# pmcgannon22/rlcard

Hardware: AMD Instinct MI355X
Metric: env-steps/s (whole node) + achieved HBM GB/s, leduc-holdem 1048576 envs/GPU (higher is better)
Workload: dtype int32

## Files before the change

rlcard_amd/csrc/cs_device.h:

```cpp
#pragma once
#include <hip/hip_runtime.h>
#include <stdint.h>
#include <type_traits>

#include "cs_prof.h"

namespace cs {

typedef uint32_t u32x4_t __attribute__((ext_vector_type(4)));
__device__ __forceinline__ void out_store16(uint4* p, const uint4& v)
{
    const u32x4_t x = {v.x, v.y, v.z, v.w};
    __builtin_nontemporal_store(x, (u32x4_t*)p);
}
template <class T>
__device__ __forceinline__ void out_store(T* p, T v)
{
    __builtin_nontemporal_store(v, p);
}

constexpr int MT_N = 624;
constexpr int MT_M = 397;
constexpr int WAVE = 64;

struct GameParams {
    int32_t num_players;
    int32_t num_decks;
    int32_t chips_for_each;
    int32_t dealer_id;
    int32_t rng_mode;
};

struct GameDefaults {
    static constexpr bool LANE_OPAQUE = true;
    static constexpr bool REWARD_OPAQUE = false;
    static constexpr bool PAYOFF_DRAWS = false;
    static constexpr int SPARSE_K = 0;
    static constexpr int MAX_POLICY = 0;
    static constexpr bool RANDOM_ACTIONS = false;
    static constexpr int DQ = 0;
    static constexpr bool OBS_DIRECT = false;
    static constexpr int RAW_SPAN_LEN = 0, RAW_SPAN_AT = 0;
};

__device__ __forceinline__ uint32_t mt_temper(uint32_t y)
{
    y ^= (y >> 11);
    y ^= (y << 7) & 0x9d2c5680u;
    y ^= (y << 15) & 0xefc60000u;
    y ^= (y >> 18);
    return y;
}

__device__ __forceinline__ uint32_t mt_temper_lo8(uint32_t y)
{
    y ^= (y >> 11);
    y ^= (y << 7) & 0x9d2c5680u;
    return y ^ (y >> 18) ^ ((y >> 3) & 0xF1u);
}

__device__ __forceinline__ uint32_t mt_mix(uint32_t cur, uint32_t nxt, uint32_t far)
{
    uint32_t y;
    asm("v_bfi_b32 %0, %1, %2, %3" : "=v"(y) : "s"(0x7fffffffu), "v"(nxt), "v"(cur));
    return far ^ (y >> 1) ^ ((0u - (nxt & 1u)) & 0x9908b0dfu);
}

template <class M>
__device__ __forceinline__ uint32_t mt_get(M mt, int k)
{
    if constexpr (std::is_pointer<M>::value) return mt[k];
    else return mt.get(k);
}
template <class M>
__device__ __forceinline__ void mt_set(M mt, int k, uint32_t v)
{
    if constexpr (std::is_pointer<M>::value) mt[k] = v;
    else mt.set(k, v);
}

template <class M>
__device__ inline void mt_init_by_array(M mt, const uint32_t* key, int klen)
{
    uint32_t prev = 19650218u;
    mt_set(mt, 0, prev);
    for (int i = 1; i < MT_N; i++) {
        prev = 1812433253u * (prev ^ (prev >> 30)) + (uint32_t)i;
        mt_set(mt, i, prev);
    }
    int i = 1, j = 0;
    prev = mt_get(mt, 0);
    for (int k = MT_N; k; k--) {
        const uint32_t v = (mt_get(mt, i) ^ ((prev ^ (prev >> 30)) * 1664525u)) + key[j] + (uint32_t)j;
        mt_set(mt, i, v);
        prev = v;
        i++;
        j++;
        if (i >= MT_N) { mt_set(mt, 0, mt_get(mt, MT_N - 1)); prev = mt_get(mt, 0); i = 1; }
        if (j >= klen) j = 0;
    }
    for (int k = MT_N - 1; k; k--) {
        const uint32_t v = (mt_get(mt, i) ^ ((prev ^ (prev >> 30)) * 1566083941u)) - (uint32_t)i;
        mt_set(mt, i, v);
        prev = v;
        i++;
        if (i >= MT_N) { mt_set(mt, 0, mt_get(mt, MT_N - 1)); prev = mt_get(mt, 0); i = 1; }
    }
    mt_set(mt, 0, 0x80000000u);
}

template <class M>
__device__ inline void mt_twist_inplace(M mt)
{
    for (int k = 0; k < MT_N - MT_M; k++) mt_set(mt, k, mt_mix(mt_get(mt, k), mt_get(mt, k + 1), mt_get(mt, k + MT_M)));
    for (int k = MT_N - MT_M; k < MT_N - 1; k++)
        mt_set(mt, k, mt_mix(mt_get(mt, k), mt_get(mt, k + 1), mt_get(mt, k + MT_M - MT_N)));
    mt_set(mt, MT_N - 1, mt_mix(mt_get(mt, MT_N - 1), mt_get(mt, 0), mt_get(mt, MT_M - 1)));
}

typedef __attribute__((address_space(1))) uint32_t gu32;
typedef __attribute__((address_space(1))) uint8_t gu8;

__device__ __forceinline__ gu32* lane_ptr(uint32_t* p, int j)
{
    const uint64_t b = (uint64_t)(uintptr_t)p;
    const uint64_t lo = (uint32_t)__builtin_amdgcn_readlane((int)(uint32_t)b, j);
    const uint64_t hi = (uint32_t)__builtin_amdgcn_readlane((int)(uint32_t)(b >> 32), j);
    return (gu32*)(uintptr_t)(lo | (hi << 32));
}

enum { STAGE_NONE = 0, STAGE_LDS = 2 };

template <int W, int PAD, int ROWS = WAVE>
struct Stage {
    static_assert(W % 16 == 0 && WAVE % (W / 4) == 0, "a staged row is copied by W / 4 lanes of one wave instruction");
    static_assert(PAD % 4 == 0, "rows are written as dwords");
    static constexpr int STRIDE = W + PAD;
    static constexpr int CHUNK = STRIDE % 16 == 0 ? 16 : (STRIDE % 8 == 0 ? 8 : 4);
    static constexpr int BYTES = ROWS * STRIDE + 16;
};

__device__ __forceinline__ void wave_sync_lds()
{
    __builtin_amdgcn_wave_barrier();
    __builtin_amdgcn_fence(__ATOMIC_RELEASE, "wavefront");
    __builtin_amdgcn_fence(__ATOMIC_ACQUIRE, "wavefront");
}

template <int W, int PAD>
__device__ __forceinline__ void stage_rows_copy(uint8_t* area, uint8_t* hbm_rows, int lane, int nvalid, bool to_lds)
{
    constexpr int STRIDE = Stage<W, PAD>::STRIDE, CH = Stage<W, PAD>::CHUNK, CPR = W / CH;
#pragma unroll
    for (int i = 0; i < CPR; i++) {
        const int q = i * WAVE + lane, row = q / CPR, col = q - row * CPR;
        if (row < nvalid) {
            uint8_t* l = area + row * STRIDE + col * CH;
            uint8_t* g = hbm_rows + (size_t)q * CH;
            if constexpr (CH == 16) {
                if (to_lds) *(uint4*)l = *(const uint4*)g;
                else *(uint4*)g = *(const uint4*)l;
            } else if constexpr (CH == 8) {
                if (to_lds) *(uint2*)l = *(const uint2*)g;
                else *(uint2*)g = *(const uint2*)l;
            } else {
                if (to_lds) *(uint32_t*)l = *(const uint32_t*)g;
                else *(uint32_t*)g = *(const uint32_t*)l;
            }
        }
    }
    wave_sync_lds();
}

__device__ __forceinline__ void philox4(uint64_t seed, uint64_t env, uint64_t blk, uint32_t (&out)[4])
{
    uint32_t c0 = (uint32_t)env, c1 = (uint32_t)(env >> 32), c2 = (uint32_t)blk, c3 = (uint32_t)(blk >> 32);
    uint32_t k0 = (uint32_t)seed, k1 = (uint32_t)(seed >> 32);
#pragma unroll
    for (int r = 0; r < 10; r++) {
        const uint32_t hi0 = __umulhi(0xD2511F53u, c0), lo0 = 0xD2511F53u * c0;
        const uint32_t hi1 = __umulhi(0xCD9E8D57u, c2), lo1 = 0xCD9E8D57u * c2;
        const uint32_t n0 = hi1 ^ c1 ^ k0, n2 = hi0 ^ c3 ^ k1;
        c0 = n0;
        c1 = lo1;
        c2 = n2;
        c3 = lo0;
        k0 += 0x9E3779B9u;
        k1 += 0xBB67AE85u;
    }
    out[0] = c0;
    out[1] = c1;
    out[2] = c2;
    out[3] = c3;
}

__device__ __forceinline__ uint32_t philox_u32(uint64_t seed, uint64_t env, uint64_t t)
{
    uint32_t w[4];
    philox4(seed, env, t >> 2, w);
    const uint32_t q = (uint32_t)t & 3u;
    return q == 0 ? w[0] : (q == 1 ? w[1] : (q == 2 ? w[2] : w[3]));
}

struct PolicyRng {
    uint32_t w0, w1, w2, w3;
    __device__ __forceinline__ uint32_t at(uint64_t seed, uint64_t env, uint64_t t, bool first)
    {
        const uint32_t q = (uint32_t)t & 3u;
        if (first || q == 0) {
            uint32_t w[4];
            philox4(seed, env, t >> 2, w);
            w0 = w[0]; w1 = w[1]; w2 = w[2]; w3 = w[3];
        }
        return q == 0 ? w0 : (q == 1 ? w1 : (q == 2 ? w2 : w3));
    }
};

__device__ __forceinline__ int pick_legal32(uint32_t legal, uint32_t r)
{
    const int count = __popc(legal);
    if (count == 0) return -1;
    int k = (int)__umulhi(r, (uint32_t)count);
    while (k--) legal &= legal - 1;
    return __builtin_ctz(legal);
}
__device__ __forceinline__ int pick_legal64(uint64_t legal, uint32_t r)
{
    const int count = __popcll(legal);
    if (count == 0) return -1;
    int k = (int)__umulhi(r, (uint32_t)count);
    while (k--) legal &= legal - 1;
    return __builtin_ctzll(legal);
}
struct Legal128 {
    uint64_t lo, hi;
};
__device__ __forceinline__ bool legal_empty(const Legal128& m) { return (m.lo | m.hi) == 0ull; }
__device__ __forceinline__ bool legal_has(const Legal128& m, int a) { return ((a < 64 ? m.lo : m.hi) >> (a & 63)) & 1ull; }
__device__ __forceinline__ int legal_lowest(const Legal128& m)
{
    return m.lo ? __builtin_ctzll(m.lo) : 64 + __builtin_ctzll(m.hi);
}
__device__ __forceinline__ int pick_legal128(const Legal128& legal, uint32_t r)
{
    const int clo = __popcll(legal.lo), count = clo + __popcll(legal.hi);
    if (count == 0) return -1;
    int k = (int)__umulhi(r, (uint32_t)count);
    const bool high = k >= clo;
    uint64_t w = high ? legal.hi : legal.lo;
    k -= high ? clo : 0;
    while (k--) w &= w - 1;
    return (high ? 64 : 0) + __builtin_ctzll(w);
}
struct Legal256 {
    uint64_t w[4];
};
__device__ __forceinline__ bool legal_empty(const Legal256& m) { return (m.w[0] | m.w[1] | m.w[2] | m.w[3]) == 0ull; }
__device__ __forceinline__ uint64_t legal_word(const Legal256& m, int k)
{
    return k == 0 ? m.w[0] : (k == 1 ? m.w[1] : (k == 2 ? m.w[2] : m.w[3]));
}
__device__ __forceinline__ bool legal_has(const Legal256& m, int a) { return (legal_word(m, a >> 6) >> (a & 63)) & 1ull; }
__device__ __forceinline__ int legal_lowest(const Legal256& m)
{
    if (m.w[0]) return __builtin_ctzll(m.w[0]);
    if (m.w[1]) return 64 + __builtin_ctzll(m.w[1]);
    if (m.w[2]) return 128 + __builtin_ctzll(m.w[2]);
    return 192 + __builtin_ctzll(m.w[3]);
}
__device__ __forceinline__ int pick_legal256(const Legal256& legal, uint32_t r)
{
    const int c0 = __popcll(legal.w[0]), c1 = c0 + __popcll(legal.w[1]), c2 = c1 + __popcll(legal.w[2]);
    const int count = c2 + __popcll(legal.w[3]);
    if (count == 0) return -1;
    int k = (int)__umulhi(r, (uint32_t)count);
    const int q = k < c0 ? 0 : (k < c1 ? 1 : (k < c2 ? 2 : 3));
    uint64_t w = legal_word(legal, q);
    k -= q == 0 ? 0 : (q == 1 ? c0 : (q == 2 ? c1 : c2));
    while (k--) w &= w - 1;
    return 64 * q + __builtin_ctzll(w);
}
template <int A>
__device__ __forceinline__ int pick_legal_small(uint32_t legal, uint32_t r)
{
    static_assert(A >= 1 && A <= 8, "small action sets");
    const uint32_t count = (uint32_t)__popc(legal);
    const uint32_t k = __umulhi(r, count);
#pragma unroll
    for (uint32_t i = 0; i + 1 < (uint32_t)A; i++) legal = i < k ? legal & (legal - 1u) : legal;
    return count == 0 ? -1 : __builtin_ctz(legal);
}

template <int ROW, int ROWS = WAVE>
struct RowWriter {
    static_assert(ROW % 4 == 0, "byte rows must be dword multiples");
    static constexpr int DW = ROW / 4;
    static constexpr int LDS_WORDS = ROWS * DW;
    static constexpr int NB = (ROW + 31) / 32;
    static constexpr int Q = (ROWS * DW) / 4;

    __device__ static __forceinline__ uint32_t expand4(uint32_t x)
    {
        return __umul24(x & 15u, 0x204081u) & 0x01010101u;
    }

    __device__ static __forceinline__ void write(uint32_t* lds, const uint32_t (&bits)[NB], uint8_t* out_span,
                                                 int lane, int nvalid, bool wide = true)
    {
        if (lane < ROWS) {
#pragma unroll
            for (int j = 0; j < DW; j++) lds[lane * DW + j] = expand4(bits[j / 8] >> (4 * (j % 8)));
        }
        write_out(lds, bits, out_span, lane, nvalid, wide);
    }
    __device__ static __forceinline__ void write_out(uint32_t* lds, const uint32_t (&)[NB], uint8_t* out_span,
                                                     int lane, int nvalid, bool wide)
    {
        __builtin_amdgcn_wave_barrier();
        __builtin_amdgcn_fence(__ATOMIC_RELEASE, "wavefront");
        __builtin_amdgcn_fence(__ATOMIC_ACQUIRE, "wavefront");
        if (wide && nvalid == ROWS && (((uintptr_t)out_span) & 15u) == 0) {
            uint4* o = (uint4*)out_span;
            const uint4* src = (const uint4*)lds;
#pragma unroll
            for (int j = 0; j < (Q + WAVE - 1) / WAVE; j++) {
                const int q = j * WAVE + lane;
                if (q < Q) out_store16(o + q, src[q]);
            }
        } else {
            uint32_t* o = (uint32_t*)out_span;
            const int total = nvalid * DW;
#pragma unroll
            for (int j = 0; j < DW; j++) {
                const int e = j * WAVE + lane;
                if (e < total) o[e] = lds[e];
            }
        }
        __builtin_amdgcn_wave_barrier();
        __builtin_amdgcn_fence(__ATOMIC_RELEASE, "wavefront");
        __builtin_amdgcn_fence(__ATOMIC_ACQUIRE, "wavefront");
    }
};

template <int ROW, int ROWS = WAVE>
struct RowWriterRaw {
    static_assert(ROW % 2 == 0, "raw rows are staged as 16-bit pieces");
    static constexpr int NW = (ROW + 3) / 4;
    static constexpr int SPAN = ROWS * ROW;
    static constexpr int LDS_WORDS = (SPAN + 3) / 4;

    __device__ static __forceinline__ void write(uint32_t* lds, const uint32_t (&words)[NW], uint8_t* out_span,
                                                 int lane, int nvalid, bool wide = true)
    {
        if (lane < ROWS) {
            if constexpr (ROW % 4 == 0) {
#pragma unroll
                for (int j = 0; j < ROW / 4; j++) lds[lane * (ROW / 4) + j] = words[j];
            } else {
                uint16_t* l16 = (uint16_t*)lds + lane * (ROW / 2);
#pragma unroll
                for (int j = 0; j < ROW / 2; j++) l16[j] = (uint16_t)(words[j / 2] >> (16 * (j & 1)));
            }
        }
        write_out(lds, out_span, lane, nvalid, wide);
// ... 88 lines not shown
```

rlcard_amd/csrc/cs_leduc.h:

```cpp
#pragma once
#include "cs_device.h"
#include "../../include/cardsim.h"

#include "cs_prof.h"

namespace cs {

struct Leduc : GameDefaults {
    static constexpr int OBS = 36, A = 4, P = 2, LB = 1, WORDS = 2, ACTION_BYTES = 1;
    static constexpr int NB = 2;
    static constexpr bool RAW_OBS = false;
    static constexpr int SCRATCH_WORDS = 0;
    static constexpr int STAGE_W = 64, STAGE_PAD = 4, STAGE_R = 12;
    static constexpr int STAGE_RF = 24;
    static constexpr int RESTAGE_B = 4;
    static constexpr int MIN_WAVES = 6;
    static constexpr int EPW = 64;
    __device__ __forceinline__ void bind(uint32_t*, const GameParams&) {}
    enum { CALL = 0, RAISE = 1, FOLD = 2, CHECK = 3 };

    int h0, h1, pub, in0, in1, r0, r1, hr, nrn, over, rc, ptr, f0, f1;

    __device__ __forceinline__ void load(const uint32_t* st, int64_t n, int64_t env)
    {
        const uint32_t w0 = st[env], w1 = st[n + env];
        h0 = w0 & 7; h1 = (w0 >> 3) & 7; pub = (w0 >> 6) & 7; in0 = (w0 >> 9) & 31; in1 = (w0 >> 14) & 31;
        r0 = (w0 >> 19) & 15; r1 = (w0 >> 23) & 15; hr = (w0 >> 27) & 3; nrn = (w0 >> 29) & 3; over = w0 >> 31;
        rc = w1 & 3; ptr = (w1 >> 2) & 1; f0 = (w1 >> 3) & 1; f1 = (w1 >> 4) & 1;
    }
    __device__ __forceinline__ void store(uint32_t* st, int64_t n, int64_t env) const
    {
        st[env] = (uint32_t)h0 | (uint32_t)h1 << 3 | (uint32_t)pub << 6 | (uint32_t)in0 << 9 | (uint32_t)in1 << 14 |
                  (uint32_t)r0 << 19 | (uint32_t)r1 << 23 | (uint32_t)hr << 27 | (uint32_t)nrn << 29 |
                  (uint32_t)over << 31;
        st[n + env] = (uint32_t)rc | (uint32_t)ptr << 2 | (uint32_t)f0 << 3 | (uint32_t)f1 << 4;
    }
    __device__ __forceinline__ void blank() { h0 = h1 = pub = in0 = in1 = r0 = r1 = hr = nrn = rc = ptr = f0 = f1 = 0; over = 1; }

    __device__ __forceinline__ int current() const { return ptr; }
    __device__ __forceinline__ bool is_over() const { return over != 0; }

    __device__ __forceinline__ uint32_t legal() const
    {
        const int mx = r0 > r1 ? r0 : r1, rp = ptr ? r1 : r0;
        uint32_t m = 0xF;
        if (hr >= 2) m &= ~(1u << RAISE);
        if (rp < mx) m &= ~(1u << CHECK);
        if (rp == mx) m &= ~(1u << CALL);
        return m;
    }

    static constexpr int MAX_POLICY = CS_POLICY_RULE_V2;
    __device__ __forceinline__ int rule_action(uint32_t policy, int player, uint32_t lg) const
    {
        const int hand = player ? h1 : h0;
        const int v1 = (lg >> RAISE) & 1u ? RAISE : ((lg >> CALL) & 1u ? CALL : ((lg >> CHECK) & 1u ? CHECK : FOLD));
        const bool pairs = rc >= 1 && ((pub ^ hand) >> 1) == 0;
        const int v2 = pairs ? ((lg >> RAISE) & 1u ? RAISE : CALL) : FOLD;
        return policy == CS_POLICY_RULE_V2 ? v2 : v1;
    }

    __device__ __forceinline__ void observe(int player, uint32_t (&bits)[NB]) const
    {
        const int my = player ? in1 : in0, hand = player ? h1 : h0;
        uint64_t b = (1ull << (hand >> 1)) | (1ull << (my + 6)) | (1ull << (in0 + in1 - my + 21));
        if (rc >= 1) b |= 1ull << ((pub >> 1) + 3);
        bits[0] = (uint32_t)b;
        bits[1] = (uint32_t)(b >> 32);
    }

    static constexpr int SPARSE_K = 4;
    __device__ __forceinline__ uint32_t observe_pos(int player, uint32_t (&pos)[4]) const
    {
        const int my = player ? in1 : in0, hand = (player ? h1 : h0) >> 1;
        pos[0] = (uint32_t)hand;
        pos[1] = (uint32_t)(rc >= 1 ? (pub >> 1) + 3 : hand);
        pos[2] = (uint32_t)(my + 6);
        pos[3] = (uint32_t)(in0 + in1 - my + 21);
        return 0;
    }

    template <class Rng>
    __device__ __forceinline__ static bool deal_swar(Rng& rng, uint32_t& code)
    {
        const uint32_t k0 = rng.staged_offset();
        const uint32_t avail = k0 < rng.sn ? rng.sn - k0 : 0u, nv = avail < 16u ? avail : 16u;
        if (nv < 6u) return false;
        const uint32_t* row = (const uint32_t*)(rng.stg + (k0 & ~3u));
        uint32_t w[5];
#pragma unroll
        for (int i = 0; i < 5; i++) w[i] = row[i];
        uint32_t m0 = 0, m1 = 0, m3 = 0;
#pragma unroll
        for (int i = 0; i < 4; i++) {
            const uint32_t x = __builtin_amdgcn_alignbyte(w[i + 1], w[i], k0 & 3u);
            const uint32_t b1 = x >> 1, b2 = x >> 2;
            const uint32_t a0 = ~(b1 & b2) & 0x01010101u;
            const uint32_t a1 = ~(b2 & (b1 | x)) & 0x01010101u;
            const uint32_t a3 = ~(x & b1) & 0x01010101u;
            m0 |= ((a0 * 0x10204080u) >> 28) << (4 * i);
            m1 |= ((a1 * 0x10204080u) >> 28) << (4 * i);
            m3 |= ((a3 * 0x10204080u) >> 28) << (4 * i);
        }
        const uint32_t valid = (1u << nv) - 1u;
        m0 &= valid;
        if (!m0) return false;
        const uint32_t p0 = __builtin_ctz(m0);
        const uint32_t r1 = m1 & valid & (0xFFFFFFFEu << p0);
        if (!r1) return false;
        const uint32_t p1 = __builtin_ctz(r1), p2 = p1 + 1;
        const uint32_t r3 = m3 & valid & (0xFFFFFFFEu << p2);
        if (!r3) return false;
        const uint32_t p5 = __builtin_ctz(r3) + 2;
        if (p5 >= nv) return false;
        const uint8_t* b = rng.stg + k0;
        const uint32_t j1 = b[p0] & 7u, j2 = b[p1] & 7u, j3 = b[p2] & 3u, s = b[p5] & 1u;
        rng.advance_by(p5 + 1);
        const uint32_t hh0 = j1, hh1 = j2 == j1 ? 5u : j2;
        const uint32_t pb = j3 == j2 ? (j1 == 4u ? 5u : 4u) : (j3 == j1 ? 5u : j3);
        code = hh0 | hh1 << 3 | pb << 6 | s << 9;
        return true;
    }

    template <class Rng>
    __device__ __forceinline__ static uint32_t draw_deal(Rng& rng)
    {
#if CS_PROF_NO_RESET
        rng.advance_by(7u);
        return 0u | 2u << 3 | 4u << 6 | (rng.pos & 1u) << 9;
#endif
        if constexpr (Rng::kMode == STAGE_LDS) {
            uint32_t code;
            if (deal_swar(rng, code)) return code;
        }
        uint32_t deck = 0x543210u;
        uint32_t q = 0, s = 0;
        auto take = [&](uint32_t b) {
            const uint32_t mx = q < 5 ? 5 - q : 1;
            const uint32_t u = b & (mx >= 4 ? 7u : (mx >= 2 ? 3u : 1u));
            if (u <= mx) {
                if (q < 5) {
                    const uint32_t ci = (deck >> (4 * mx)) & 15u, cj = (deck >> (4 * u)) & 15u, x = ci ^ cj;
                    deck ^= (x << (4 * mx)) | (x << (4 * u));
                } else {
                    s = u;
                }
                q++;
            }
        };
        if constexpr (Rng::kMode == STAGE_LDS) {
            const uint32_t k0 = rng.staged_offset();
            uint32_t k = k0;
            while (q < 6 && k < rng.sn) {
                const uint32_t sh = k & 3u;
                const uint32_t w = *(const uint32_t*)(rng.stg + (k - sh)) >> (8 * sh);
#pragma unroll
                for (uint32_t t = 0; t < 4; t++)
                    if (t < 4 - sh && q < 6 && k < rng.sn) {
                        take((w >> (8 * t)) & 255u);
                        k++;
                    }
            }
            rng.advance_by(k - k0);
        }
        while (q < 6) take(rng.next8());
        return ((deck >> 20) & 15u) | ((deck >> 16) & 15u) << 3 | ((deck >> 12) & 15u) << 6 | s << 9;
    }

    __device__ __forceinline__ void deal_blinds(int s)
    {
        in0 = s == 0 ? 1 : 2;
        in1 = s == 0 ? 2 : 1;
        ptr = s;
        r0 = in0; r1 = in1;
        hr = 0; nrn = 0; rc = 0; f0 = 0; f1 = 0; over = 0;
    }

    template <class Rng>
    __device__ __forceinline__ void reset(Rng& rng)
    {
        const uint32_t e0 = draw_deal(rng);
        h0 = (int)(e0 & 7u);
        h1 = (int)((e0 >> 3) & 7u);
        pub = (int)((e0 >> 6) & 7u);
        deal_blinds((int)((e0 >> 9) & 1u));
    }

    template <class Rng>
    __device__ __forceinline__ void step(int a, Rng&)
    {
        const uint32_t lg = legal();
        if (a < 0 || a > 3 || !((lg >> a) & 1u)) a = ((lg >> CHECK) & 1u) ? CHECK : FOLD;
        const int mx = r0 > r1 ? r0 : r1, rp = ptr ? r1 : r0, ra = rc == 0 ? 2 : 4;
        int add = 0, nr = rp;
        if (a == CALL) { add = mx - rp; nr = mx; nrn += 1; }
        else if (a == RAISE) { add = mx - rp + ra; nr = mx + ra; hr += 1; nrn = 1; }
        else if (a == FOLD) { if (ptr) f1 = 1; else f0 = 1; }
        else { nrn += 1; }
        if (ptr) { in1 += add; r1 = nr; } else { in0 += add; r0 = nr; }
        ptr ^= 1;
        if (ptr ? f1 : f0) ptr ^= 1;
        if (nrn >= 2) {
            rc += 1;
            hr = 0; nrn = 0; r0 = 0; r1 = 0;
        }
        over = (f0 + f1 == 1) || rc >= 2;
    }

    __device__ __forceinline__ void payoffs(float (&r)[P]) const
    {
        int w0, w1;
        if (f0 || f1) { w0 = !f0; w1 = !f1; }
        else {
            const int pr = pub >> 1, k0 = h0 >> 1, k1 = h1 >> 1;
            if (k0 == pr) { w0 = 1; w1 = 0; }
            else if (k1 == pr) { w0 = 0; w1 = 1; }
            else { w0 = k0 >= k1; w1 = k1 >= k0; }
        }
        const float tot = (float)(in0 + in1), each = (w0 & w1) ? tot * 0.5f : tot;
        r[0] = (w0 ? each - (float)in0 : -(float)in0) * 0.5f;
        r[1] = (w1 ? each - (float)in1 : -(float)in1) * 0.5f;
    }
};

}
```

rlcard_amd/csrc/cs_prof.h:

```cpp
#pragma once

#ifndef CS_PROF_NO_OBS
#define CS_PROF_NO_OBS 0
#endif
#ifndef CS_PROF_NO_SMALL
#define CS_PROF_NO_SMALL 0
#endif
#ifndef CS_PROF_NO_RESET
#define CS_PROF_NO_RESET 0
#endif
#ifndef CS_PROF_NO_EVAL
#define CS_PROF_NO_EVAL 0
#endif
#ifndef CS_PROF_NO_DEAL9
#define CS_PROF_NO_DEAL9 0
#endif
#ifndef CS_PROF_NO_TRACK
#define CS_PROF_NO_TRACK 0
#endif
#ifndef CS_PROF_NO_SKIP
#define CS_PROF_NO_SKIP 0
#endif
#ifndef CS_PROF_MIXED_WRITER
#define CS_PROF_MIXED_WRITER 0
#endif
#ifndef CS_PROF_MIXED_NT
#define CS_PROF_MIXED_NT 0
#endif
#ifndef CS_PROF_BRIDGE_WAVES
#define CS_PROF_BRIDGE_WAVES 0
#endif
#ifndef CS_PROF_MIXED16_NT
#define CS_PROF_MIXED16_NT 0
#endif
#ifndef CS_PROF_SCOUT_MASK
#define CS_PROF_SCOUT_MASK 0
#endif
#ifndef CS_PROF_SCOUT_WAVES
#define CS_PROF_SCOUT_WAVES 0
#endif
#ifndef CS_PROF_DDZ
#define CS_PROF_DDZ 0
#endif
```

rlcard_amd/csrc/cs_skeleton.h:

```cpp
#pragma once
#include <cstddef>
#include <type_traits>

#include "cs_device.h"
#include "cs_ring.h"
#include "cs_engine.h"
#include "cs_dq.h"

namespace cs {

constexpr int BLOCK = 256;
constexpr int WAVES_PER_BLOCK = BLOCK / WAVE;

template <class G>
using legal_t = std::conditional_t<(G::A > 128), Legal256, std::conditional_t<(G::A > 64), Legal128, uint64_t>>;

struct LaneCtx {
    int lane, wid;
    int64_t env, wave_first;
    int nvalid;
    bool valid;
};

template <int EPW = WAVE>
// ... 428 lines not shown
    CS_SMEM(G);
    const LaneCtx c = lane_ctx(n);
    RingLane<> m = ring_lane(mt, ctl, c);
    G g;
    g.bind(scratch_of<G>(scr[c.wid], c.lane), prm);
    g.blank();
    float r[G::P];
#pragma unroll
    for (int k = 0; k < G::P; k++) r[k] = 0.f;
    bool done = false;
    if (c.valid) {
        g.load(st, n, c.env);
        if (g.is_over()) {
            game_reset(g, m, st, n, c.env);
        } else {
            g.step(actions[c.env], m);
            done = g.is_over();
            if (done) game_payoffs(g, r, m);
        }
    }
    refill(m, c.lane, flags & 1);
    uint32_t bits[G::NB];
    const int p = g.current();
    g.observe(p, bits);
    if (out.obs) emit_obs<G>(lds[c.wid], bits, (uint8_t*)out.obs, c.wave_first, flags, c);
    if (c.valid) {
        if (out.legal) emit_legal<G>((uint8_t*)out.legal, c.env, g.legal());
        if (out.player) ((uint8_t*)out.player)[c.env] = (uint8_t)p;
        if (out.reward) emit_reward<G>((float*)out.reward, c.env, r);
        if (out.done) ((uint8_t*)out.done)[c.env] = (uint8_t)done;
        g.store(st, n, c.env);
        ctl[c.env] = m.ctl_word();
    }
    step_record<G>(rec, st, n, c);
}

template <class G>
__global__ __launch_bounds__(BLOCK) void k_observe(const uint32_t* st, int64_t n, int player, cs_step_out out,
                                                    GameParams prm, StepRecord rec)
{
    CS_SMEM(G);
    const LaneCtx c = lane_ctx(n);
    G g;
    g.bind(scratch_of<G>(scr[c.wid], c.lane), prm);
    g.blank();
    if (c.valid) g.load(st, n, c.env);
    uint32_t bits[G::NB];
    g.observe(player, bits);
    if (out.obs) emit_obs<G>(lds[c.wid], bits, (uint8_t*)out.obs, c.wave_first, 0, c);
    if (c.valid) {
        if (out.legal) emit_legal<G>((uint8_t*)out.legal, c.env, g.legal());
        if (out.player) ((uint8_t*)out.player)[c.env] = (uint8_t)g.current();
        if (out.done) ((uint8_t*)out.done)[c.env] = (uint8_t)g.is_over();
    }
    step_record<G>(rec, st, n, c);
}

struct RolloutArgs {
    uint32_t* mt;
    uint32_t* ctl;
    uint32_t* st;
    int64_t n;
    uint64_t seed, t0, env_base;
    cs_traj_out out;
    GameParams prm;
    uint32_t* sctl;
    uint8_t* sbuf;
    int32_t T, flags;
    uint32_t seats;
    uint32_t pad_;
};
typedef const __attribute__((address_space(4))) RolloutArgs* RolloutArgsK;
static_assert(std::is_standard_layout<RolloutArgs>::value && std::is_trivially_copyable<RolloutArgs>::value,
              "RolloutArgs is copied into the kernarg segment bytewise");
static_assert(offsetof(RolloutArgs, mt) == 0 && alignof(RolloutArgs) == 8 && sizeof(RolloutArgs) % 8 == 0,
              "RolloutArgs: first kernarg at offset 0, 8-byte aligned");

template <class G, bool POL = false>
__global__ __launch_bounds__(BLOCK, G::MIN_WAVES) void k_rollout(RolloutArgs args)
{
    RolloutArgsK ak = (RolloutArgsK)__builtin_amdgcn_kernarg_segment_ptr();
    auto arg = [&]() -> const RolloutArgs& {
        asm volatile("" : "+s"(ak));
        return *(const RolloutArgs*)ak;
    };
    uint32_t* const mt = args.mt;
    uint32_t* const ctl = args.ctl;
    uint32_t* const st = args.st;
    const int64_t n = args.n;
    const int T = args.T, flags = args.flags;
    const GameParams prm = args.prm;
    uint32_t* const sctl = args.sctl;
    uint8_t* const sbuf = args.sbuf;
    CS_SMEM_ROWS(G, G::EPW);
    __shared__ __attribute__((aligned(16))) uint8_t stage[WAVES_PER_BLOCK][StageBytes<G>::value];
    const LaneCtx c = lane_ctx<G::EPW>(n);
    RingLane<STAGE_LDS> m = ring_lane<STAGE_LDS>(mt, ctl, c);
    const bool staged = !(flags & 3);
    uint8_t* rows = sbuf + c.wave_first * G::STAGE_W;
    if (staged) {
        if (c.valid && ((ctl[c.env] >> 17) & 1u)) {
            const uint32_t w = sctl[c.env];
            m.sp = w & 0xFFFFu;
            m.sn = w >> 16;
        }
        stage_rows_copy<G::STAGE_W, G::STAGE_PAD>(stage[c.wid], rows, c.lane, c.nvalid, true);
    }
    constexpr int DQ = DqOf<G>::value, DQW = DqOf<G>::words;
    __shared__ uint32_t dql[DQ > 0 ? WAVES_PER_BLOCK * G::EPW * DQW : 1];
    DqMem q{};
    if constexpr (DQ > 0) {
        q = DqMem{dql + (c.wid * G::EPW + (c.lane < G::EPW ? c.lane : 0)) * DQW, 1};
        if (c.valid) {
#pragma unroll
            for (int w = 0; w < DQW; w++) q.set(w, st[(int64_t)(G::GW + w) * n + c.env]);
        }
    }
    G g;
    g.bind(scratch_of<G>(scr[c.wid], c.lane), prm);
    g.blank();
    if (c.valid) {
        g.load(st, n, c.env);
        if (g.is_over()) {
            if constexpr (DQ > 0) dq_reset(g, m, q);
            else g.reset(m);
        }
    }
    refill(m, c.lane, flags & 1);
    if (staged) restage<G>(m, stage[c.wid], c.lane, c.valid);
    PolicyRng pol;
    const uint64_t genv0 = args.env_base + (uint64_t)c.env;
    for (int t = 0; t < T; t++) {
        const RolloutArgs& A = arg();
        LaneCtx cl = c;
        if constexpr (G::LANE_OPAQUE) {
            int ol = c.lane;
            asm volatile("" : "+v"(ol));
            cl.lane = ol;
            cl.env = c.wave_first + ol;
        }
        const cs_traj_out& out = A.out;
        uint8_t* obs = (uint8_t*)out.obs;
        uint8_t* legal = (uint8_t*)out.legal;
        uint8_t* player = (uint8_t*)out.player;
        float* reward = (float*)out.reward;
        uint8_t* done_o = (uint8_t*)out.done;
        const uint64_t seed = A.seed, t0 = A.t0;

        const int64_t rowbase = (int64_t)t * n;
        const int p = g.current();
        const legal_t<G> lg = g.legal();
        uint32_t bits[G::NB];
        g.observe(p, bits);
        const uint32_t pr = pol.at(seed, genv0, t0 + (uint64_t)t, t == 0);
        int a;
        static_assert(G::A <= 256, "the policy pick takes a legal mask of one, two or four 64-bit words");
        if constexpr (G::A > 128) a = pick_legal256(lg, pr);
        else if constexpr (G::A > 64) a = pick_legal128(lg, pr);
        else if constexpr (G::A <= 8) a = pick_legal_small<G::A>((uint32_t)lg, pr);
        else if constexpr (G::A <= 32) a = pick_legal32((uint32_t)lg, pr);
        else a = pick_legal64(lg, pr);
        if constexpr (POL) {
            const uint32_t pid = (A.seats >> (8 * p)) & 0xFFu;
            int ra;
            if constexpr (G::A <= 32) ra = g.rule_action(pid, p, (uint32_t)lg);
            else ra = g.rule_action(pid, p, lg, pr);
            a = pid == (uint32_t)CS_POLICY_RANDOM ? a : ra;
        }
#if !CS_PROF_NO_OBS
        if constexpr (G::SPARSE_K > 0) {
            uint32_t pos[G::SPARSE_K];
            const uint32_t tail = g.observe_pos(p, pos);
            row_write_sparse<G::OBS, G::EPW, G::SPARSE_K, G::RAW_OBS>(
                lds[c.wid], pos, obs + (rowbase + c.wave_first) * G::OBS, cl.lane, c.nvalid, !(flags & 4), tail);
        } else {
            emit_obs<G, G::EPW>(lds[c.wid], bits, obs, rowbase + c.wave_first, flags, cl);
        }
#endif
        uint32_t zr = 0;
        asm volatile("" : "+v"(zr));
        float r[G::P];
#pragma unroll
        for (int k = 0; k < G::P; k++) r[k] = __uint_as_float(zr);
        bool done = false;
        if (c.valid) {
            const int64_t row = rowbase + cl.env;
#if !CS_PROF_NO_SMALL
            emit_legal<G>(legal, row, lg);
            out_store(player + row, (uint8_t)p);
#endif
            if constexpr (G::ACTION_BYTES == 1) out_store((uint8_t*)out.action + row, (uint8_t)a);
            else out_store((int16_t*)out.action + row, (int16_t)a);
            g.step(a, m);
            done = g.is_over();
            if (done) {
                game_payoffs(g, r, m);
                if (out.final_obs) {
#pragma unroll
                    for (int q = 0; q < G::P; q++) {
                        uint32_t fb[G::NB];
                        g.observe(q, fb);
                        write_obs_direct<G>((uint8_t*)out.final_obs + (row * G::P + q) * G::OBS, fb);
                    }
                }
            }
#if !CS_PROF_NO_SMALL
            emit_reward<G>(reward, row, r);
            out_store(done_o + row, (uint8_t)done);
#endif
            if constexpr (DQ == 0) {
                if (done) g.reset(m);
            }
        }
        if constexpr (DQ > 0) {
            constexpr uint32_t CM = (1u << DqOf<G>::cb) - 1u;
            if (__ballot(c.valid && done && (q.get(0) & CM) == 0u)) {
                if (c.valid && (q.get(0) & CM) < (uint32_t)DQ) dq_push(g, m, q);
            }
            if (c.valid && done) dq_reset(g, m, q);
        }
        refill(m, cl.lane, flags & 1);
        if (staged) restage<G>(m, stage[c.wid], cl.lane, c.valid);
    }
    bool keep = false;
    if (staged) {
        stage_rows_copy<G::STAGE_W, G::STAGE_PAD>(stage[c.wid], rows, c.lane, c.nvalid, false);
        keep = true;
    }
    if (c.valid) {
        g.store(st, n, c.env);
        if constexpr (DQ > 0) {
#pragma unroll
            for (int w = 0; w < DQW; w++) st[(int64_t)(G::GW + w) * n + c.env] = q.get(w);
        }
        ctl[c.env] = m.ctl_word() | ((uint32_t)keep << 17);
        if (keep) sctl[c.env] = m.sp | (m.sn << 16);
    }
}

template <class G>
__global__ __launch_bounds__(BLOCK) void k_policy_actions(const uint32_t* st, int64_t n, int policy, uint64_t seed,
                                                           uint64_t t, uint64_t env_base, int32_t* actions,
                                                           GameParams prm)
{
    const int64_t env = (int64_t)blockIdx.x * BLOCK + threadIdx.x;
    uint32_t* lane_scratch = nullptr;
    if constexpr (G::SCRATCH_WORDS > 0) {
        __shared__ uint32_t scr[WAVES_PER_BLOCK][Scratch<G>::WORDS];
        lane_scratch = scratch_of<G>(scr[threadIdx.x / WAVE], threadIdx.x & (WAVE - 1));
    }
    if (env >= n) return;
    G g;
    g.bind(lane_scratch, prm);
    g.blank();
    g.load(st, n, env);
    int a = -1;
    if (!g.is_over()) {
        if constexpr (G::A > 128) {
            static_assert(G::MAX_POLICY == 0, "rule policies take masks of at most two words");
            a = pick_legal256(g.legal(), philox_u32(seed, env_base + (uint64_t)env, t));
        } else if constexpr (G::A > 64) {
            const Legal128 lg = g.legal();
            const uint32_t pr = philox_u32(seed, env_base + (uint64_t)env, t);
            if constexpr (G::MAX_POLICY > 0) {
                if (policy == CS_POLICY_RANDOM) a = pick_legal128(lg, pr);
                else a = g.rule_action((uint32_t)policy, g.current(), lg, pr);
            } else {
                a = pick_legal128(lg, pr);
            }
        } else if constexpr (G::A <= 32) {
            const uint32_t lg = (uint32_t)g.legal();
            if (policy == CS_POLICY_RANDOM) a = pick_legal_small<G::A>(lg, philox_u32(seed, env_base + (uint64_t)env, t));
            else a = g.rule_action((uint32_t)policy, g.current(), lg);
        } else {
            const uint64_t lg = g.legal();
            const uint32_t pr = philox_u32(seed, env_base + (uint64_t)env, t);
            if constexpr (G::MAX_POLICY > 0) {
                if (policy == CS_POLICY_RANDOM) a = pick_legal64(lg, pr);
                else a = g.rule_action((uint32_t)policy, g.current(), lg, pr);
            } else {
                a = pick_legal64(lg, pr);
            }
        }
    }
    actions[env] = a;
}

static inline GameParams params_of(const Buffers& b)
{
    return GameParams{b.num_players, b.num_decks, b.chips_for_each, b.dealer_id, b.rng_mode};
}
static inline dim3 grid_for(int64_t n, int epw = WAVE)
{
    const int64_t per = (int64_t)WAVES_PER_BLOCK * epw;
    return dim3((unsigned)((n + per - 1) / per));
}

template <class G>
static hipError_t seed_g(const Buffers& b, const uint32_t* keys, const int32_t* klen, int64_t first, int64_t count,
                         hipStream_t s)
{
    hipLaunchKernelGGL(k_seed<G>, grid_for(count), dim3(BLOCK), 0, s, b.mt, b.ctl, b.state, b.n, keys, klen, first,
                       count, b.kernel_flags, params_of(b));
    return hipGetLastError();
}
template <class G>
static hipError_t reset_g(const Buffers& b, const cs_step_out& o, hipStream_t s)
{
    hipLaunchKernelGGL(k_reset<G>, grid_for(b.n), dim3(BLOCK), 0, s, b.mt, b.ctl, b.state, b.n, o, b.kernel_flags,
                       params_of(b), b.rec);
    return hipGetLastError();
}
template <class G>
static hipError_t step_g(const Buffers& b, const int32_t* a, const cs_step_out& o, hipStream_t s)
{
    hipLaunchKernelGGL(k_step<G>, grid_for(b.n), dim3(BLOCK), 0, s, b.mt, b.ctl, b.state, b.n, a, o, b.kernel_flags,
                       params_of(b), b.rec);
    return hipGetLastError();
}
template <class G>
static hipError_t observe_g(const Buffers& b, int32_t p, const cs_step_out& o, hipStream_t s)
{
    hipLaunchKernelGGL(k_observe<G>, grid_for(b.n), dim3(BLOCK), 0, s, b.state, b.n, p, o, params_of(b), b.rec);
    return hipGetLastError();
}
template <class G>
static hipError_t rollout_g(const Buffers& b, int32_t T, uint64_t seed, uint64_t t0, uint64_t env_base,
                            const cs_traj_out& o, hipStream_t s)
{
    const RolloutArgs a{b.mt, b.ctl, b.state, b.n, seed, t0, env_base, o, params_of(b), b.sctl, b.sbuf, T, b.kernel_flags};
    hipLaunchKernelGGL(k_rollout<G>, grid_for(b.n, G::EPW), dim3(BLOCK), 0, s, a);
    return hipGetLastError();
}

template <class G>
static hipError_t rollout_policy_g(const Buffers& b, int32_t T, uint64_t seed, uint64_t t0, uint64_t env_base,
                                   uint32_t seats, const cs_traj_out& o, hipStream_t s)
{
    const RolloutArgs a{b.mt, b.ctl, b.state, b.n, seed, t0, env_base, o, params_of(b), b.sctl, b.sbuf, T, b.kernel_flags,
                        seats, 0u};
    hipLaunchKernelGGL((k_rollout<G, true>), grid_for(b.n, G::EPW), dim3(BLOCK), 0, s, a);
    return hipGetLastError();
}
template <class G>
static hipError_t policy_actions_g(const Buffers& b, int32_t policy, uint64_t seed, uint64_t t, uint64_t env_base,
                                   int32_t* actions, hipStream_t s)
{
    hipLaunchKernelGGL(k_policy_actions<G>, dim3((unsigned)((b.n + BLOCK - 1) / BLOCK)), dim3(BLOCK), 0, s, b.state,
                       b.n, policy, seed, t, env_base, actions, params_of(b));
    return hipGetLastError();
}

template <class G>
static void fill_info(cs_game_info* info)
{
    info->obs_dim = G::OBS;
    info->num_actions = G::A;
    info->num_players = G::P;
    info->legal_bytes = G::LB;
    info->action_bytes = G::ACTION_BYTES;
    info->state_words = G::WORDS;
    info->action_feature_dim = G::A;
    info->rng_period = (int32_t)RING;
    info->deal_queue_depth = DqOf<G>::value;
    info->game_words = G::WORDS - DqOf<G>::words;
    info->envs_per_wave = G::EPW;
}

template <class G>
static const GameOps* ops_of()
{
    static const GameOps ops = [] {
        GameOps o{seed_g<G>, reset_g<G>, step_g<G>, observe_g<G>, rollout_g<G>, {}, G::STAGE_W,
                  RING_ENV_WORDS, false, false};
        fill_info<G>(&o.info);
// ... 14 lines not shown
```

Baseline: 75.19 billion.

## Branchless Leduc rules, 64-bit-window deal, wide-multiply Philox, profiling knockouts

Moves the Leduc step, legal, payoff and blind logic into a shared host/device rules header and rewrites them as branchless select chains. The staged deal scan now packs the 16-byte window into nibbles and searches all positions with one 64-bit mask per card instead of four per-dword loops with early exits. Philox can use a 64-bit product to get the high and low halves together, and Leduc enables this by default. It also adds compile-time profiling switches that stub out philox, pick, step, refill and restage, all off by default. The aim is less divergence and fewer ALU ops per step, with the risk that the branchless forms do more work on average.

```diff
diff --git a/rlcard_amd/csrc/cs_device.h b/rlcard_amd/csrc/cs_device.h
--- a/rlcard_amd/csrc/cs_device.h
+++ b/rlcard_amd/csrc/cs_device.h
@@ -35,6 +35,7 @@
     static constexpr bool LANE_OPAQUE = true;
     static constexpr bool REWARD_OPAQUE = false;
     static constexpr bool PAYOFF_DRAWS = false;
+    static constexpr bool PHILOX_WIDE = false;
     static constexpr int SPARSE_K = 0;
     static constexpr int MAX_POLICY = 0;
     static constexpr bool RANDOM_ACTIONS = false;
@@ -172,14 +173,22 @@
     wave_sync_lds();
 }
 
+template <bool WIDE = false>
 __device__ __forceinline__ void philox4(uint64_t seed, uint64_t env, uint64_t blk, uint32_t (&out)[4])
 {
     uint32_t c0 = (uint32_t)env, c1 = (uint32_t)(env >> 32), c2 = (uint32_t)blk, c3 = (uint32_t)(blk >> 32);
     uint32_t k0 = (uint32_t)seed, k1 = (uint32_t)(seed >> 32);
 #pragma unroll
     for (int r = 0; r < 10; r++) {
-        const uint32_t hi0 = __umulhi(0xD2511F53u, c0), lo0 = 0xD2511F53u * c0;
-        const uint32_t hi1 = __umulhi(0xCD9E8D57u, c2), lo1 = 0xCD9E8D57u * c2;
+        uint32_t hi0, lo0, hi1, lo1;
+        if constexpr (WIDE) {
+            const uint64_t p0 = (uint64_t)0xD2511F53u * c0, p1 = (uint64_t)0xCD9E8D57u * c2;
+            hi0 = (uint32_t)(p0 >> 32); lo0 = (uint32_t)p0;
+            hi1 = (uint32_t)(p1 >> 32); lo1 = (uint32_t)p1;
+        } else {
+            hi0 = __umulhi(0xD2511F53u, c0); lo0 = 0xD2511F53u * c0;
+            hi1 = __umulhi(0xCD9E8D57u, c2); lo1 = 0xCD9E8D57u * c2;
+        }
         const uint32_t n0 = hi1 ^ c1 ^ k0, n2 = hi0 ^ c3 ^ k1;
         c0 = n0;
         c1 = lo1;
@@ -204,12 +213,13 @@
 
 struct PolicyRng {
     uint32_t w0, w1, w2, w3;
+    template <bool WIDE = false>
     __device__ __forceinline__ uint32_t at(uint64_t seed, uint64_t env, uint64_t t, bool first)
     {
         const uint32_t q = (uint32_t)t & 3u;
         if (first || q == 0) {
             uint32_t w[4];
-            philox4(seed, env, t >> 2, w);
+            philox4<WIDE>(seed, env, t >> 2, w);
             w0 = w[0]; w1 = w[1]; w2 = w[2]; w3 = w[3];
         }
         return q == 0 ? w0 : (q == 1 ? w1 : (q == 2 ? w2 : w3));
diff --git a/rlcard_amd/csrc/cs_leduc.h b/rlcard_amd/csrc/cs_leduc.h
--- a/rlcard_amd/csrc/cs_leduc.h
+++ b/rlcard_amd/csrc/cs_leduc.h
@@ -3,10 +3,11 @@
 #include "../../include/cardsim.h"
 
 #include "cs_prof.h"
+#include "cs_leduc_rules.h"
 
 namespace cs {
 
-struct Leduc : GameDefaults {
+struct Leduc : GameDefaults, leduc::State {
     static constexpr int OBS = 36, A = 4, P = 2, LB = 1, WORDS = 2, ACTION_BYTES = 1;
     static constexpr int NB = 2;
     static constexpr bool RAW_OBS = false;
@@ -17,9 +18,8 @@
     static constexpr int MIN_WAVES = 6;
     static constexpr int EPW = 64;
     __device__ __forceinline__ void bind(uint32_t*, const GameParams&) {}
-    enum { CALL = 0, RAISE = 1, FOLD = 2, CHECK = 3 };
-
-    int h0, h1, pub, in0, in1, r0, r1, hr, nrn, over, rc, ptr, f0, f1;
+    enum { CALL = leduc::CALL, RAISE = leduc::RAISE, FOLD = leduc::FOLD, CHECK = leduc::CHECK };
+    static constexpr bool PHILOX_WIDE = !CS_PROF_PHILOX_NARROW;
 
     __device__ __forceinline__ void load(const uint32_t* st, int64_t n, int64_t env)
     {
@@ -40,15 +40,11 @@
     __device__ __forceinline__ int current() const { return ptr; }
     __device__ __forceinline__ bool is_over() const { return over != 0; }
 
-    __device__ __forceinline__ uint32_t legal() const
-    {
-        const int mx = r0 > r1 ? r0 : r1, rp = ptr ? r1 : r0;
-        uint32_t m = 0xF;
-        if (hr >= 2) m &= ~(1u << RAISE);
-        if (rp < mx) m &= ~(1u << CHECK);
-        if (rp == mx) m &= ~(1u << CALL);
-        return m;
-    }
+#if CS_PROF_NO_STEP
+    __device__ __forceinline__ uint32_t legal() const { return 0xFu; }
+#else
+    __device__ __forceinline__ uint32_t legal() const { return leduc::legal(*this); }
+#endif
 
     static constexpr int MAX_POLICY = CS_POLICY_RULE_V2;
     __device__ __forceinline__ int rule_action(uint32_t policy, int player, uint32_t lg) const
@@ -81,45 +77,17 @@
     }
 
     template <class Rng>
-    __device__ __forceinline__ static bool deal_swar(Rng& rng, uint32_t& code)
+    __device__ __forceinline__ static bool deal_staged(const Rng& rng, uint32_t& code, uint32_t& used)
     {
         const uint32_t k0 = rng.staged_offset();
         const uint32_t avail = k0 < rng.sn ? rng.sn - k0 : 0u, nv = avail < 16u ? avail : 16u;
-        if (nv < 6u) return false;
-        const uint32_t* row = (const uint32_t*)(rng.stg + (k0 & ~3u));
-        uint32_t w[5];
+        uint32_t w[5] = {0u, 0u, 0u, 0u, 0u};
+        if (nv >= 6u) {
+            const uint32_t* row = (const uint32_t*)(rng.stg + (k0 & ~3u));
 #pragma unroll
-        for (int i = 0; i < 5; i++) w[i] = row[i];
-        uint32_t m0 = 0, m1 = 0, m3 = 0;
-#pragma unroll
-        for (int i = 0; i < 4; i++) {
-            const uint32_t x = __builtin_amdgcn_alignbyte(w[i + 1], w[i], k0 & 3u);
-            const uint32_t b1 = x >> 1, b2 = x >> 2;
-            const uint32_t a0 = ~(b1 & b2) & 0x01010101u;
-            const uint32_t a1 = ~(b2 & (b1 | x)) & 0x01010101u;
-            const uint32_t a3 = ~(x & b1) & 0x01010101u;
-            m0 |= ((a0 * 0x10204080u) >> 28) << (4 * i);
-            m1 |= ((a1 * 0x10204080u) >> 28) << (4 * i);
-            m3 |= ((a3 * 0x10204080u) >> 28) << (4 * i);
+            for (int i = 0; i < 5; i++) w[i] = row[i];
         }
-        const uint32_t valid = (1u << nv) - 1u;
-        m0 &= valid;
-        if (!m0) return false;
-        const uint32_t p0 = __builtin_ctz(m0);
-        const uint32_t r1 = m1 & valid & (0xFFFFFFFEu << p0);
-        if (!r1) return false;
-        const uint32_t p1 = __builtin_ctz(r1), p2 = p1 + 1;
-        const uint32_t r3 = m3 & valid & (0xFFFFFFFEu << p2);
-        if (!r3) return false;
-        const uint32_t p5 = __builtin_ctz(r3) + 2;
-        if (p5 >= nv) return false;
-        const uint8_t* b = rng.stg + k0;
-        const uint32_t j1 = b[p0] & 7u, j2 = b[p1] & 7u, j3 = b[p2] & 3u, s = b[p5] & 1u;
-        rng.advance_by(p5 + 1);
-        const uint32_t hh0 = j1, hh1 = j2 == j1 ? 5u : j2;
-        const uint32_t pb = j3 == j2 ? (j1 == 4u ? 5u : 4u) : (j3 == j1 ? 5u : j3);
-        code = hh0 | hh1 << 3 | pb << 6 | s << 9;
-        return true;
+        return leduc::deal_window(w, k0 & 3u, nv, code, used);
     }
 
     template <class Rng>
@@ -130,9 +98,18 @@
         return 0u | 2u << 3 | 4u << 6 | (rng.pos & 1u) << 9;
 #endif
         if constexpr (Rng::kMode == STAGE_LDS) {
-            uint32_t code;
-            if (deal_swar(rng, code)) return code;
+            uint32_t code, used;
+            if (deal_staged(rng, code, used)) {
+                rng.advance_by(used);
+                return code;
+            }
         }
+        return draw_deal_bytes(rng);
+    }
+
+    template <class Rng>
+    __device__ __forceinline__ static uint32_t draw_deal_bytes(Rng& rng)
+    {
         uint32_t deck = 0x543210u;
         uint32_t q = 0, s = 0;
         auto take = [&](uint32_t b) {
@@ -167,14 +144,7 @@
         return ((deck >> 20) & 15u) | ((deck >> 16) & 15u) << 3 | ((deck >> 12) & 15u) << 6 | s << 9;
     }
 
-    __device__ __forceinline__ void deal_blinds(int s)
-    {
-        in0 = s == 0 ? 1 : 2;
-        in1 = s == 0 ? 2 : 1;
-        ptr = s;
-        r0 = in0; r1 = in1;
-        hr = 0; nrn = 0; rc = 0; f0 = 0; f1 = 0; over = 0;
-    }
+    __device__ __forceinline__ void deal_blinds(int s) { leduc::deal_blinds(*this, s); }
 
     template <class Rng>
     __device__ __forceinline__ void reset(Rng& rng)
@@ -186,41 +156,24 @@
         deal_blinds((int)((e0 >> 9) & 1u));
     }
 
+#if CS_PROF_NO_STEP
     template <class Rng>
     __device__ __forceinline__ void step(int a, Rng&)
     {
-        const uint32_t lg = legal();
-        if (a < 0 || a > 3 || !((lg >> a) & 1u)) a = ((lg >> CHECK) & 1u) ? CHECK : FOLD;
-        const int mx = r0 > r1 ? r0 : r1, rp = ptr ? r1 : r0, ra = rc == 0 ? 2 : 4;
-        int add = 0, nr = rp;
-        if (a == CALL) { add = mx - rp; nr = mx; nrn += 1; }
-        else if (a == RAISE) { add = mx - rp + ra; nr = mx + ra; hr += 1; nrn = 1; }
-        else if (a == FOLD) { if (ptr) f1 = 1; else f0 = 1; }
-        else { nrn += 1; }
-        if (ptr) { in1 += add; r1 = nr; } else { in0 += add; r0 = nr; }
         ptr ^= 1;
-        if (ptr ? f1 : f0) ptr ^= 1;
-        if (nrn >= 2) {
-            rc += 1;
-            hr = 0; nrn = 0; r0 = 0; r1 = 0;
-        }
-        over = (f0 + f1 == 1) || rc >= 2;
+        over = a & 1;
     }
-
     __device__ __forceinline__ void payoffs(float (&r)[P]) const
     {
-        int w0, w1;
-        if (f0 || f1) { w0 = !f0; w1 = !f1; }
-        else {
-            const int pr = pub >> 1, k0 = h0 >> 1, k1 = h1 >> 1;
-            if (k0 == pr) { w0 = 1; w1 = 0; }
-            else if (k1 == pr) { w0 = 0; w1 = 1; }
-            else { w0 = k0 >= k1; w1 = k1 >= k0; }
-        }
-        const float tot = (float)(in0 + in1), each = (w0 & w1) ? tot * 0.5f : tot;
-        r[0] = (w0 ? each - (float)in0 : -(float)in0) * 0.5f;
-        r[1] = (w1 ? each - (float)in1 : -(float)in1) * 0.5f;
+        r[0] = ptr ? 0.5f : -0.5f;
+        r[1] = -r[0];
     }
+#else
+    template <class Rng>
+    __device__ __forceinline__ void step(int a, Rng&) { leduc::step(*this, a); }
+
+    __device__ __forceinline__ void payoffs(float (&r)[P]) const { leduc::payoffs(*this, r); }
+#endif
 };
 
 }
diff --git a/rlcard_amd/csrc/cs_leduc_rules.h b/rlcard_amd/csrc/cs_leduc_rules.h
--- /dev/null
+++ b/rlcard_amd/csrc/cs_leduc_rules.h
@@ -0,0 +1,128 @@
+#pragma once
+#include <stdint.h>
+
+#if defined(__HIPCC__) || defined(__CUDACC__)
+#define CS_LEDUC_HD __host__ __device__ __forceinline__
+#else
+#define CS_LEDUC_HD inline
+#endif
+
+namespace cs {
+namespace leduc {
+
+enum { CALL = 0, RAISE = 1, FOLD = 2, CHECK = 3 };
+
+struct State {
+    int h0, h1, pub, in0, in1, r0, r1, hr, nrn, over, rc, ptr, f0, f1;
+};
+
+CS_LEDUC_HD uint32_t legal(const State& s)
+{
+    const int mx = s.r0 > s.r1 ? s.r0 : s.r1, rp = s.ptr ? s.r1 : s.r0;
+    const uint32_t m = s.hr >= 2 ? 0xFu & ~(1u << RAISE) : 0xFu;
+    return m & (rp == mx ? ~(1u << CALL) : ~(1u << CHECK));
+}
+
+CS_LEDUC_HD void step(State& s, int a)
+{
+    const uint32_t lg = legal(s);
+    const bool playable = (uint32_t)a <= 3u && ((lg >> ((uint32_t)a & 3u)) & 1u) != 0u;
+    a = playable ? a : (((lg >> CHECK) & 1u) ? CHECK : FOLD);
+    const int p = s.ptr;
+    const int mx = s.r0 > s.r1 ? s.r0 : s.r1, rp = p ? s.r1 : s.r0, ra = s.rc == 0 ? 2 : 4;
+    const bool call = a == CALL, raise = a == RAISE, fold = a == FOLD;
+    const int nr = ((call || raise) ? mx : rp) + (raise ? ra : 0);
+    const int add = nr - rp;
+    s.hr += raise ? 1 : 0;
+    s.nrn = raise ? 1 : s.nrn + (fold ? 0 : 1);
+    s.f0 |= (fold && !p) ? 1 : 0;
+    s.f1 |= (fold && p) ? 1 : 0;
+    s.in0 += p ? 0 : add;
+    s.in1 += p ? add : 0;
+    s.r0 = p ? s.r0 : nr;
+    s.r1 = p ? nr : s.r1;
+    s.ptr = (p ? s.f0 : s.f1) ? p : (p ^ 1);
+    const bool next_round = s.nrn >= 2;
+    s.rc += next_round ? 1 : 0;
+    s.hr = next_round ? 0 : s.hr;
+    s.nrn = next_round ? 0 : s.nrn;
+    s.r0 = next_round ? 0 : s.r0;
+    s.r1 = next_round ? 0 : s.r1;
+    s.over = ((s.f0 + s.f1 == 1) || s.rc >= 2) ? 1 : 0;
+}
+
+CS_LEDUC_HD void payoffs(const State& s, float (&r)[2])
+{
+    const int pr = s.pub >> 1, k0 = s.h0 >> 1, k1 = s.h1 >> 1;
+    const bool folded = (s.f0 | s.f1) != 0;
+    const bool p0 = k0 == pr, p1 = k1 == pr;
+    const bool s0 = p0 || (!p1 && k0 >= k1), s1 = !p0 && (p1 || k1 >= k0);
+    const bool w0 = folded ? !s.f0 : s0, w1 = folded ? !s.f1 : s1;
+    const float a0 = (float)s.in0, a1 = (float)s.in1;
+    const float tot = (float)(s.in0 + s.in1), each = (w0 && w1) ? tot * 0.5f : tot;
+    r[0] = (w0 ? each - a0 : -a0) * 0.5f;
+    r[1] = (w1 ? each - a1 : -a1) * 0.5f;
+}
+
+CS_LEDUC_HD void deal_blinds(State& g, int s)
+{
+    g.in0 = 1 + s;
+    g.in1 = 1 + (s ^ 1);
+    g.ptr = s;
+    g.r0 = g.in0;
+    g.r1 = g.in1;
+    g.hr = 0; g.nrn = 0; g.rc = 0; g.f0 = 0; g.f1 = 0; g.over = 0;
+}
+
+
+CS_LEDUC_HD uint32_t pack_nibbles(uint32_t x, uint32_t y)
+{
+    x &= 0x07070707u;
+    y &= 0x07070707u;
+    x |= x >> 4;
+    y |= y >> 4;
+    return (x & 0xFFu) | ((x >> 8) & 0xFF00u) | ((y & 0xFFu) << 16) | ((y << 8) & 0xFF000000u);
+}
+CS_LEDUC_HD uint32_t first_set64(uint64_t v) { return (uint32_t)__builtin_ctzll(v | 1ull << 63); }
+CS_LEDUC_HD uint32_t window_dword(uint32_t lo, uint32_t hi, uint32_t sh)
+{
+#if defined(__HIP_DEVICE_COMPILE__)
+    return __builtin_amdgcn_alignbyte(hi, lo, sh);
+#else
+    return (uint32_t)(((uint64_t)hi << 32 | lo) >> (8u * (sh & 3u)));
+#endif
+}
+CS_LEDUC_HD bool deal_window(const uint32_t (&w)[5], uint32_t sh, uint32_t nv, uint32_t& code, uint32_t& used)
+{
+    const uint32_t n0 = pack_nibbles(window_dword(w[0], w[1], sh), window_dword(w[1], w[2], sh));
+    const uint32_t n1 = pack_nibbles(window_dword(w[2], w[3], sh), window_dword(w[3], w[4], sh));
+    const uint64_t below = nv >= 16u ? ~0ull : (1ull << (4u * nv)) - 1ull;
+    const uint32_t v0 = (uint32_t)below & 0x11111111u, v1 = (uint32_t)(below >> 32) & 0x11111111u;
+    const uint32_t b10 = n0 >> 1, b20 = n0 >> 2, b11 = n1 >> 1, b21 = n1 >> 2;
+    auto both = [](uint32_t lo, uint32_t hi) { return (uint64_t)lo | (uint64_t)hi << 32; };
+    const uint64_t a0 = both(~(b10 & b20) & v0, ~(b11 & b21) & v1);
+    const uint64_t a1 = both(~(b20 & (b10 | n0)) & v0, ~(b21 & (b11 | n1)) & v1);
+    const uint64_t a3 = both(~(n0 & b10) & v0, ~(n1 & b11) & v1);
+    bool ok = nv >= 6u && a0 != 0ull;
+    const uint32_t q0 = first_set64(a0);
+    const uint64_t c1 = a1 & (~1ull << q0);
+    const uint32_t q1 = first_set64(c1);
+    ok = ok && c1 != 0ull && q1 < 60u;
+    const uint32_t q2 = (q1 + 4u) & 63u;
+    const uint64_t c3 = a3 & (~1ull << q2);
+    ok = ok && c3 != 0ull;
+    const uint32_t q3 = first_set64(c3);
+    const uint32_t p5 = (q3 >> 2) + 2u;
+    ok = ok && p5 < nv;
+    const uint64_t nib = (uint64_t)n0 | (uint64_t)n1 << 32;
+    const uint32_t j1 = (uint32_t)(nib >> q0) & 7u, j2 = (uint32_t)(nib >> q1) & 7u;
+    const uint32_t j3 = (uint32_t)(nib >> q2) & 3u, s = (uint32_t)(nib >> ((q3 + 8u) & 63u)) & 1u;
+    const uint32_t hh0 = j1, hh1 = j2 == j1 ? 5u : j2;
+    const uint32_t pb = j3 == j2 ? (j1 == 4u ? 5u : 4u) : (j3 == j1 ? 5u : j3);
+    code = hh0 | hh1 << 3 | pb << 6 | s << 9;
+    used = p5 + 1u;
+    return ok;
+}
+
+}
+}
diff --git a/rlcard_amd/csrc/cs_prof.h b/rlcard_amd/csrc/cs_prof.h
--- a/rlcard_amd/csrc/cs_prof.h
+++ b/rlcard_amd/csrc/cs_prof.h
@@ -8,6 +8,24 @@
 #endif
 #ifndef CS_PROF_NO_RESET
 #define CS_PROF_NO_RESET 0
+#endif
+#ifndef CS_PROF_NO_PHILOX
+#define CS_PROF_NO_PHILOX 0
+#endif
+#ifndef CS_PROF_PHILOX_NARROW
+#define CS_PROF_PHILOX_NARROW 0
+#endif
+#ifndef CS_PROF_NO_PICK
+#define CS_PROF_NO_PICK 0
+#endif
+#ifndef CS_PROF_NO_STEP
+#define CS_PROF_NO_STEP 0
+#endif
+#ifndef CS_PROF_NO_REFILL
+#define CS_PROF_NO_REFILL 0
+#endif
+#ifndef CS_PROF_NO_RESTAGE
+#define CS_PROF_NO_RESTAGE 0
 #endif
 #ifndef CS_PROF_NO_EVAL
 #define CS_PROF_NO_EVAL 0
diff --git a/rlcard_amd/csrc/cs_skeleton.h b/rlcard_amd/csrc/cs_skeleton.h
--- a/rlcard_amd/csrc/cs_skeleton.h
+++ b/rlcard_amd/csrc/cs_skeleton.h
@@ -604,9 +604,19 @@
         const legal_t<G> lg = g.legal();
         uint32_t bits[G::NB];
         g.observe(p, bits);
-        const uint32_t pr = pol.at(seed, genv0, t0 + (uint64_t)t, t == 0);
+#if CS_PROF_NO_PHILOX
+        const uint32_t pr = ((uint32_t)genv0 ^ (uint32_t)seed) * 0x9E3779B1u + (uint32_t)(t0 + (uint64_t)t) * 0x85EBCA6Bu;
+#else
+        const uint32_t pr = pol.template at<G::PHILOX_WIDE>(seed, genv0, t0 + (uint64_t)t, t == 0);
+#endif
         int a;
         static_assert(G::A <= 256, "the policy pick takes a legal mask of one, two or four 64-bit words");
+#if CS_PROF_NO_PICK
+        if constexpr (G::A <= 8) {
+            const uint32_t m = (uint32_t)lg;
+            a = (pr >> 31) ? 31 - __builtin_clz(m | 1u) : __builtin_ctz(m | 0x80000000u);
+        } else
+#endif
         if constexpr (G::A > 128) a = pick_legal256(lg, pr);
         else if constexpr (G::A > 64) a = pick_legal128(lg, pr);
         else if constexpr (G::A <= 8) a = pick_legal_small<G::A>((uint32_t)lg, pr);
@@ -671,8 +681,22 @@
             }
             if (c.valid && done) dq_reset(g, m, q);
         }
+#if CS_PROF_NO_REFILL
+        if (m.needs_refill()) m.lat = (m.lat + (uint32_t)RING_GEN) & SLOT_MASK;
+#else
         refill(m, cl.lane, flags & 1);
+#endif
+#if CS_PROF_NO_RESTAGE
+        if (staged) {
+            const uint32_t k = m.staged_offset();
+            if (c.valid && (k >= m.sn || m.sn - k < (uint32_t)G::STAGE_R)) {
+                m.sp = m.pos & ~3u;
+                m.sn = (uint32_t)G::STAGE_W;
+            }
+        }
+#else
         if (staged) restage<G>(m, stage[c.wid], cl.lane, c.valid);
+#endif
     }
     bool keep = false;
     if (staged) {
```

Result: no change. 75.70 billion, median of 2 (+0.7%).
